# jpedro1992/gym-loadbalancing

Hardware: AMD Instinct MI355X
Metric: env-steps/sec (whole node) at 1M envs, 1/2/4/8 GPUs; % HBM roofline (higher is better)
Workload: dtype f64

## Files before the change

### gym-loadbalancing_amd/csrc/lbk8s_env.hip

```cpp

#include <hip/hip_runtime.h>

#include <cstdint>
#include <cstdio>
#include <cstdlib>
#include <algorithm>
#include <cstring>
#include <string>
#include <type_traits>

#include "lbk8s.h"
#include "lbk8s_common.h"
#include "lbk8s_host.h"
#include "lbk8s_slice.h"
#include "lbk8s_tpe.h"
#include "lbk8s_rollout.h"
#include "lbk8s_lean_launch.h"

namespace lbk {

__global__ void k_luts(double* lat_lut, double* cpu_lut) {
    int row = blockIdx.x * blockDim.x + threadIdx.x;
    if (row < LAT_ROWS) {
        double v = (double)row;
// ... 96 lines not shown
        case LB_FIELD_ENDPOINT_LATENCY: v = lat_of(p, p.lat0[i], ed); break;
        case LB_FIELD_ENDPOINT_CPU: v = cpu_of(p, em, ed); break;
        case LB_FIELD_ENDPOINT_TOPOLOGY_LATENCY: v = (double)topo_val(topo, em_zone(em), s.rz); break;
        case LB_FIELD_ENDPOINT_ZONE_CPU_CAPACITY: v = (double)zcap_val(zc, em_zone(em)); break;
        case LB_FIELD_ENDPOINT_ZONE: v = (double)em_zone(em); break;
        case LB_FIELD_ENDPOINT_NODE: v = (double)em_node(em); break;
        default: v = (double)ed_j(ed); break;
        }
        out[env * p.E + e] = v;
    }
}

__global__ void k_stats(Params p, double* out) {
    int64_t env = (int64_t)blockIdx.x * blockDim.x + threadIdx.x;
    if (env >= p.B) return;
    write_stats_row(p, out + env * LB_ST_K, sc_unpack(p.sc[env]), p.acc2[env], p.acc3[env], p.total[env],
                    p.sum_lat[env], p.sum_cpu[env], p.sum_hi[env]);
}

__global__ void k_status(Params p, uint32_t* flags) {
    int64_t env = (int64_t)blockIdx.x * blockDim.x + threadIdx.x;
    uint32_t f = 0;
    if (env < p.B) {
        Scal s = sc_unpack(p.sc[env]);
        if (s.bad) f |= LB_STATUS_BAD_ACTION;
        if (!s.reset_done) f |= LB_STATUS_NOT_RESET;
    }
    if (f) atomicOr(flags, f);
}

thread_local std::string g_err;
#ifdef LB_EXPERIMENTS
int g_rollout_variant = 0;
#else
constexpr int g_rollout_variant = 0;
#endif

int fail(const char* msg) {
    g_err = msg;
    return -1;
}

Geo geometry(const lb_config* c, int64_t B) {
    Geo g;
    const int E = c->num_endpoints;
    g.tpe = E <= TPE_E;
    if (g.tpe && B > 0 && B < WIDE_SLICE_MAX_B) g.tpe = false;
    if (E <= TPE_E && c->geometry == LB_GEOMETRY_TPE) g.tpe = true;
    if (c->geometry == LB_GEOMETRY_SLICE) g.tpe = false;
    if (g.tpe) {
        g.W = 1;
        g.EPL = 1;
        g.EP = E;
    } else {
        const bool wide = B < WIDE_SLICE_MAX_B;
        if (wide) {
            g.W = E <= 16 ? 16 : E <= 32 ? 32 : 64;
            g.EPL = E <= 64 ? 1 : E <= 128 ? 2 : 4;
        } else {
            g.W = E <= 64 ? 16 : E <= 128 ? 32 : 64;
            g.EPL = E <= 16 ? 1 : E <= 32 ? 2 : 4;
        }
        g.EP = g.W * g.EPL;
    }
    g.NZW = (c->num_nodes + 31) / 32;
    return g;
}

uint64_t align_up(uint64_t x) { return (x + 255) & ~(uint64_t)255; }

Offsets offsets(const lb_config* c, int64_t B) {
    Geo g = geometry(c, B);
    Offsets o;
    uint64_t x = 0;
    auto take = [&](uint64_t bytes) { uint64_t r = x; x = align_up(x + bytes); return r; };
    o.lat_lut = take((uint64_t)LAT_ROWS * JCAP * 8);
    o.cpu_lut = take((uint64_t)CPU_ROWS * JCAP * 8);
    const uint64_t BE = (uint64_t)B * g.EP;
    o.lat0 = take(BE * 8);
    o.emeta = take(BE * 4);
    o.edyn = take(BE * 4);
    o.t = take(B * 8);
    o.sc = take(B * 8);
    o.topo = take(B * 8);
    o.zcap = take(B * 8);
    o.nzone = take((uint64_t)B * g.NZW * 8);
    o.acc2 = take(B * 8);
    o.acc3 = take(B * 8);
    o.sum_lat = take(B * 8);
    o.sum_cpu = take(B * 8);
    o.sum_hi = take(B * 4);
    o.total = take(B * 8);
    o.last_r = take(B * 8);
    o.rew64 = take(B * 8);
    o.rec = take(g.tpe ? (uint64_t)B * RO_REC_BYTES : 0);
    o.end = x;
    return o;
}

double initial_last_reward(const lb_config* c) {
    switch (c->reward_fn) {
    case LB_REWARD_NAIVE: return 1.0;
    case LB_REWARD_LATENCY: return -(0.0 + 0.0);
    case LB_REWARD_FAIRNESS: return 1.0 - 0.0;
    default: {
        volatile double cur = ((0.0 + 0.0) - 2.0) / 998.0;
        volatile double cpu = (1.0 - 1.0) / 99.0;
        volatile double a = c->latency_weight * (1.0 - cur);
        volatile double b = c->cpu_weight * (1.0 - cpu);
        volatile double g = c->gini_weight * (1.0 - 0.0);
        volatile double ab = a + b;
        return ab + g;
    }
    }
}

int validate(const lb_config* c) {
    if (!c) return fail("lb_config is NULL");
    if (c->num_endpoints < 1 || c->num_endpoints > EMAX) return fail("num_endpoints must be in [1, 256]");
    if (c->num_zones < 4)
        return fail("IndexError: num_zones < 4 (zone ids are drawn in [0,4), loadbalancer_k8s_env.py:354)");
    if (c->num_nodes < 24)
        return fail("IndexError: num_nodes < 24 (endpoint hosts are drawn in [0,24), loadbalancer_k8s_env.py:380)");
    if (c->num_nodes > 32 * NZW_MAX) return fail("num_nodes must be <= 256");
    if (c->episode_length < 1 || c->episode_length > CMAX) return fail("episode_length must be in [1, 1023]");
    if (c->reward_fn < 0 || c->reward_fn > 3) return fail("unknown reward_fn");
    if (c->rng_mode != LB_RNG_PHILOX && c->rng_mode != LB_RNG_TRACE) return fail("unknown rng_mode");
    if (c->geometry < LB_GEOMETRY_AUTO || c->geometry > LB_GEOMETRY_SLICE) return fail("unknown geometry");
// ... 81 lines not shown
int rollout_kernel(const lb_config* c, int64_t B, int32_t steps, bool outputs_all) {
    const Geo g = geometry(c, B);
    if (!g.tpe) return LB_ROLLOUT_SLICE;
    if (g.NZW > 2) return LB_ROLLOUT_STEPS;
    const bool pre = c->auto_reset && c->episode_length >= steps;
    if (!pre) return LB_ROLLOUT_TPE;
    const uint64_t lim = 0xFFFFFFFFull;
    const int R = c->num_endpoints + (c->rejection_allowed ? 1 : 0);
    const bool img_fits = offsets(c, B).end <= lim && (uint64_t)B * LB_ST_K * 8 <= lim;
    const bool lean_fits = img_fits && (uint64_t)B * R * 32 <= lim;
    const bool lean_shape = (c->num_endpoints == 8 && R == 9 && c->num_nodes <= 32) ||
                            (c->num_endpoints == 6 && R == 7 && c->num_nodes <= 64);
    if (lean_fits && lean_shape && B % 64 == 0 && B > SMALL_TPE_MAX_B && outputs_all &&
        g_rollout_variant == 0)
        return steps <= LEAN_SPLIT_MAX_K ? LB_ROLLOUT_LEAN_SPLIT : LB_ROLLOUT_LEAN;
    if (img_fits && g_rollout_variant != 3) return LB_ROLLOUT_IMG;
    return LB_ROLLOUT_TPE;
}

template <typename F>
void with_policy(int policy, bool flag, F f) {
    auto two = [&](auto kind) {
        if (flag) f(kind, std::true_type{});
        else f(kind, std::false_type{});
    };
    switch (policy) {
    case LB_POLICY_TOPOLOGY_GREEDY: two(std::integral_constant<int, LB_POLICY_TOPOLOGY_GREEDY>{}); break;
    case LB_POLICY_ZONE_CPU_GREEDY: two(std::integral_constant<int, LB_POLICY_ZONE_CPU_GREEDY>{}); break;
    case LB_POLICY_ENDPOINT_CPU_GREEDY: two(std::integral_constant<int, LB_POLICY_ENDPOINT_CPU_GREEDY>{}); break;
    default: two(std::integral_constant<int, LB_POLICY_RANDOM>{}); break;
    }
}

}

using namespace lbk;

extern "C" {

int lb_abi_version(void) { return LBK8S_ABI_VERSION; }


#ifdef LB_EXPERIMENTS
int lbx_set_rollout_variant(int v) { g_rollout_variant = v; return 0; }
#endif
#ifdef LB_TIMELINE
int lbx_set_timeline(uint64_t* buf) {
    int r = hipMemcpyToSymbol(HIP_SYMBOL(g_timeline), &buf, sizeof(buf)) == hipSuccess ? 0 : -1;
    r |= lbx_set_timeline_lean_0(buf) | lbx_set_timeline_lean_1(buf) | lbx_set_timeline_lean_2(buf) |
         lbx_set_timeline_lean_3(buf);
    return r;
}
#endif

const char* lb_last_error(void) { return g_err.c_str(); }

int lb_validate_config(const lb_config* cfg) { return validate(cfg); }

int lb_state_bytes(const lb_config* cfg, int64_t num_envs, uint64_t* out_bytes) {
    if (int r = validate(cfg)) return r;
    if (num_envs < 1 || !out_bytes) return fail("num_envs must be >= 1 and out_bytes non-NULL");
    *out_bytes = offsets(cfg, num_envs).end;
    return 0;
}

int lb_init(void* state, const lb_config* cfg, int64_t num_envs, const lb_trace* trace, void* stream) {
    if (int r = validate(cfg)) return r;
    if (!state || num_envs < 1) return fail("state NULL or num_envs < 1");
    const bool tr = cfg->rng_mode == LB_RNG_TRACE;
    if (tr && (!trace || !trace->t0)) return fail("trace mode: lb_init needs trace->t0");
    Params p = make_params(state, cfg, num_envs);
    if (tr) p.tr = *trace;
    hipStream_t s = (hipStream_t)stream;
    hipLaunchKernelGGL(k_luts, dim3((LAT_ROWS + CPU_ROWS + 127) / 128), dim3(128), 0, s, p.lat_lut, p.cpu_lut);
    if (int r = check_launch()) return r;
    hipLaunchKernelGGL(k_init, dim3(env_blocks(num_envs)), dim3(BLOCK), 0, s, p, tr ? 1 : 0);
    return check_launch();
}

int lb_reset(void* state, const lb_config* cfg, int64_t num_envs, const uint8_t* reset_mask,
             float* obs_out, const lb_trace* trace, void* stream) {
    if (int r = validate(cfg)) return r;
    if (!state || num_envs < 1) return fail("state NULL or num_envs < 1");
    const bool tr = cfg->rng_mode == LB_RNG_TRACE;
    if (tr && (!trace || !trace->reset_lat0 || !trace->reset_topo || !trace->reset_ntype ||
               !trace->reset_nzone || !trace->reset_ncpu || !trace->reset_enode || !trace->reset_x1 ||
               !trace->reset_x2 || !trace->reset_r || !trace->reset_n))
        return fail("trace mode: lb_reset needs every reset_* trace array");
    Params p = make_params(state, cfg, num_envs);
    if (tr) p.tr = *trace;
    p.obs = obs_out;
    p.reset_mask = reset_mask;
    Geo g = geometry(cfg, num_envs);
    hipStream_t s = (hipStream_t)stream;
    if (g.tpe) {
        if (num_envs <= SMALL_TPE_MAX_B) {
            const unsigned nb = (unsigned)((num_envs + 63) / 64);
            if (tr) hipLaunchKernelGGL((k_reset_tpe<true, 64>), dim3(nb), dim3(64), 0, s, p);
            else hipLaunchKernelGGL((k_reset_tpe<false, 64>), dim3(nb), dim3(64), 0, s, p);
            return check_launch();
        }
        if (tr) hipLaunchKernelGGL(k_reset_tpe<true>, dim3(env_blocks(num_envs)), dim3(BLOCK), 0, s, p);
        else hipLaunchKernelGGL(k_reset_tpe<false>, dim3(env_blocks(num_envs)), dim3(BLOCK), 0, s, p);
        return check_launch();
    }
    LB_DISPATCH_SLICE(g.W, g.EPL, {
// ... 36 lines not shown
        } else if (tr) {
            hipLaunchKernelGGL((k_step_tpe<true, false>), dim3(env_blocks(num_envs)), dim3(BLOCK), 0, s, p);
        } else if (recompute) {
            hipLaunchKernelGGL((k_step_tpe<false, true>), dim3(env_blocks(num_envs)), dim3(BLOCK), 0, s, p);
        } else {
            hipLaunchKernelGGL((k_step_tpe<false, false>), dim3(env_blocks(num_envs)), dim3(BLOCK), 0, s, p);
        }
        return check_launch();
    }
    LB_DISPATCH_SLICE(g.W, g.EPL, {
        const unsigned nb = slice_blocks(num_envs, W);
        if (tr) hipLaunchKernelGGL((k_step_slice<W, EPL, true>), dim3(nb), dim3(BLOCK), 0, s, p);
        else hipLaunchKernelGGL((k_step_slice<W, EPL, false>), dim3(nb), dim3(BLOCK), 0, s, p);
    });
    return check_launch();
}

int lb_reward64(void* state, const lb_config* cfg, int64_t num_envs, double** out) {
    if (int r = validate(cfg)) return r;
    if (!state || num_envs < 1 || !out) return fail("state/out NULL or num_envs < 1");
    *out = make_params(state, cfg, num_envs).rew64;
    return 0;
}

int lb_rollout_kernel(const lb_config* cfg, int64_t num_envs, int32_t steps, int32_t outputs_all,
                      int32_t* kernel_out) {
    if (int r = validate(cfg)) return r;
    if (num_envs < 1 || steps < 0 || !kernel_out) return fail("num_envs < 1, steps < 0 or kernel_out NULL");
    if (cfg->rng_mode != LB_RNG_PHILOX) return fail("lb_rollout draws in Philox mode only");
    *kernel_out = rollout_kernel(cfg, num_envs, steps, outputs_all != 0);
    return 0;
}

int lb_rollout(void* state, const lb_config* cfg, int64_t num_envs, int32_t policy, int32_t steps,
               float* obs_out, float* reward_out, uint8_t* done_out, int32_t* actions_out,
               float* terminal_obs_out, double* ep_stats_out, void* stream) {
    if (int r = validate(cfg)) return r;
    if (!state || num_envs < 1) return fail("state NULL or num_envs < 1");
    if (cfg->rng_mode != LB_RNG_PHILOX) return fail("lb_rollout draws in Philox mode only");
    if (policy < 0 || policy > LB_POLICY_REWARD_GREEDY) return fail("unknown policy kind");
    if (steps < 0) return fail("steps must be >= 0");
    const bool k8s = policy > LB_POLICY_RANDOM;
    Geo g = geometry(cfg, num_envs);
    hipStream_t s = (hipStream_t)stream;
    if (g.tpe && g.NZW <= 2) {
        Params p = make_params(state, cfg, num_envs);
        p.obs = obs_out;
        p.reward = reward_out;
        p.done = done_out;
        p.term_obs = terminal_obs_out;
        p.ep_stats = ep_stats_out;
        const bool small = num_envs <= SMALL_TPE_MAX_B;
        const dim3 grid(small ? (unsigned)((num_envs + 63) / 64) : env_blocks(num_envs)), block(small ? 64 : BLOCK);
        const bool pre = cfg->auto_reset && cfg->episode_length >= steps;
        if (k8s) return launch_rollout_k8s(p, g, policy, (int)steps, pre, actions_out, s);
        const int rk = rollout_kernel(cfg, num_envs, steps, obs_out && reward_out && done_out && terminal_obs_out &&
                                                                ep_stats_out);
        if (rk == LB_ROLLOUT_LEAN || rk == LB_ROLLOUT_LEAN_SPLIT) {
            const bool naive = p.reward_fn == LB_REWARD_NAIVE, act = actions_out != nullptr;
            with_policy(policy, p.E == 8, [&](auto kind, auto e8) {
                constexpr int KIND = decltype(kind)::value, ET = decltype(e8)::value ? 8 : 6, RT = ET + 1,
                              NZW = decltype(e8)::value ? 1 : 2;
                if (naive && act) launch_lean<KIND, ET, RT, NZW, true, true>(p, num_envs, (int)steps, actions_out, s);
                else if (naive) launch_lean<KIND, ET, RT, NZW, true, false>(p, num_envs, (int)steps, actions_out, s);
                else if (act) launch_lean<KIND, ET, RT, NZW, false, true>(p, num_envs, (int)steps, actions_out, s);
                else launch_lean<KIND, ET, RT, NZW, false, false>(p, num_envs, (int)steps, actions_out, s);
            });
            return check_launch();
        }
        if (rk == LB_ROLLOUT_IMG) {
            const bool e8 = p.E == 8 && p.R == 9;
            with_policy(policy, small, [&](auto kind, auto sm) {
                constexpr int KIND = decltype(kind)::value, NB = decltype(sm)::value ? 64 : BLOCK;
                if (e8) hipLaunchKernelGGL((k_rollout_img<NB, KIND, 8, 9, 4>), grid, block, 0, s, p, (int)steps, actions_out);
                else hipLaunchKernelGGL((k_rollout_img<NB, KIND, 0, 0, 4>), grid, block, 0, s, p, (int)steps, actions_out);
            });
            return check_launch();
        }
        with_policy(policy, small, [&](auto kind, auto sm) {
            constexpr int KIND = decltype(kind)::value, NB = decltype(sm)::value ? 64 : BLOCK;
            if (pre) hipLaunchKernelGGL((k_rollout_tpe<NB, KIND, true>), grid, block, 0, s, p, (int)steps, actions_out);
            else hipLaunchKernelGGL((k_rollout_tpe<NB, KIND, false>), grid, block, 0, s, p, (int)steps, actions_out);
        });
        return check_launch();
    }
    if (g.tpe) {
        if (policy != LB_POLICY_RANDOM && !actions_out)
            return fail("lb_rollout on the thread-per-env layout needs actions_out for a greedy policy");
        const int64_t R = cfg->num_endpoints + (cfg->rejection_allowed ? 1 : 0);
        for (int k = 0; k < steps; ++k) {
            int32_t* act = actions_out ? actions_out + k * num_envs : nullptr;
            if (act)
                if (int r = lb_policy(state, cfg, num_envs, policy, act, stream)) return r;
            if (int r = lb_step(state, cfg, num_envs, act, obs_out ? obs_out + k * num_envs * R * 8 : nullptr,
                                reward_out ? reward_out + k * num_envs : nullptr,
                                done_out ? done_out + k * num_envs : nullptr, terminal_obs_out, ep_stats_out,
                                nullptr, stream))
                return r;
        }
// ... 73 lines not shown
```

### gym-loadbalancing_amd/csrc/lbk8s_host.h

```cpp
#pragma once

#include <hip/hip_runtime.h>

#include <cstdint>
#include <string>

#include "lbk8s.h"
#include "lbk8s_common.h"

namespace lbk {

extern thread_local std::string g_err;
int fail(const char* msg);
int check_launch();
int validate(const lb_config* c);

struct Geo {
    bool tpe;
    int W, EPL, EP, NZW;
};

constexpr int64_t WIDE_SLICE_MAX_B = 32768;
constexpr int64_t SMALL_TPE_MAX_B = 65536;

Geo geometry(const lb_config* c, int64_t B = 0);

struct Offsets {
    uint64_t lat_lut, cpu_lut, lat0, emeta, edyn, t, sc, topo, zcap, nzone, acc2, acc3, sum_lat,
        sum_cpu, sum_hi, total, last_r, rew64, rec, end;
};

Offsets offsets(const lb_config* c, int64_t B);
Params make_params(void* state, const lb_config* c, int64_t B);

#define LB_DISPATCH_SLICE(W_, EPL_, BODY)                                         \
    do {                                                                          \
        if (W_ == 16 && EPL_ == 1) { constexpr int W = 16, EPL = 1; BODY; }       \
        else if (W_ == 16 && EPL_ == 2) { constexpr int W = 16, EPL = 2; BODY; }  \
        else if (W_ == 16 && EPL_ == 4) { constexpr int W = 16, EPL = 4; BODY; }  \
        else if (W_ == 32 && EPL_ == 4) { constexpr int W = 32, EPL = 4; BODY; }  \
        else if (W_ == 32 && EPL_ == 1) { constexpr int W = 32, EPL = 1; BODY; }  \
        else if (W_ == 64 && EPL_ == 1) { constexpr int W = 64, EPL = 1; BODY; }  \
        else if (W_ == 64 && EPL_ == 2) { constexpr int W = 64, EPL = 2; BODY; }  \
        else if (W_ == 64 && EPL_ == 4) { constexpr int W = 64, EPL = 4; BODY; }  \
        else return fail("unsupported geometry");                                 \
    } while (0)

unsigned slice_blocks(int64_t B, int W);
unsigned env_blocks(int64_t B);
int device_cus();

int launch_policy_reward_greedy(const Params& p, const Geo& g, int32_t* actions_out, hipStream_t s);
int launch_rollout_k8s(const Params& p, const Geo& g, int policy, int steps, bool pre, int32_t* actions_out,
                       hipStream_t s);

unsigned ds_grid_spread(int64_t groups);

}
```

### gym-loadbalancing_amd/csrc/lbk8s_lean.h

```cpp
#pragma once

#include "lbk8s_rollout.h"

namespace lbk {

typedef __amdgpu_buffer_rsrc_t Rsrc;
typedef uint32_t u32x2 __attribute__((ext_vector_type(2)));
typedef uint32_t u32x4 __attribute__((ext_vector_type(4)));

__device__ __forceinline__ Rsrc rsrc_of(const void* base) {
    return __builtin_amdgcn_make_buffer_rsrc(const_cast<void*>(base), (short)0, -1, 0x00020000);
}
constexpr int BUF_NT = 2;

#define LB_GUARD_S(...) asm volatile("" : "+s"(__VA_ARGS__))
#define LB_GUARD_V(...) asm volatile("" : "+v"(__VA_ARGS__))

__device__ __forceinline__ double buf_ld_f64(Rsrc r, uint32_t off) {
    return __builtin_bit_cast(double, __builtin_amdgcn_raw_buffer_load_b64(r, off, 0, 0));
}
__device__ __forceinline__ uint4 buf_ld_u128(Rsrc r, uint32_t off) {
    const u32x4 v = __builtin_amdgcn_raw_buffer_load_b128(r, off, 0, 0);
    return make_uint4(v.x, v.y, v.z, v.w);
}
// ... 429 lines not shown
            ++cep;
        }
        if (k + 1 < K) split_draws<KIND>(p, env0 + lane, cep, cs, sst, (k + 1) & 1, lane);
        block_lds_sync();
        float4 v[CW][P];
        uint32_t rw[CW], dn[CW], ac[CW];
#pragma unroll
        for (int c = 0; c < CW; ++c) {
#pragma unroll
            for (int it = 0; it < P; ++it) v[c][it] = lean_piece<P>(simg[c], lane, it, h);
            rw[c] = sst[192 * c + lane];
            dn[c] = sst[192 * c + 64 + lane];
            ac[c] = ACT ? sst[192 * c + 128 + lane] : 0u;
        }
        block_lds_sync();
        const Rsrc out = rsrc_of(p.obs + (int64_t)k * p.B * (P / 2) * 8);
        const Rsrc rwo = rsrc_of(p.reward + (int64_t)k * p.B), dno = rsrc_of(p.done + (int64_t)k * p.B);
#pragma unroll
        for (int c = 0; c < CW; ++c) {
            const uint32_t envi = (uint32_t)(env0 + 64 * c + lane);
            const uint32_t obs_wave = (uint32_t)((env0 + 64 * c) * P * 16);
#pragma unroll
            for (int it = 0; it < P; ++it)
                buf_st_f4<BUF_NT>(v[c][it], out, (uint32_t)lane * 16u + obs_wave + 1024u * (uint32_t)it);
            __builtin_amdgcn_raw_buffer_store_b32(rw[c], rwo, envi * 4u, 0, BUF_NT);
            __builtin_amdgcn_raw_buffer_store_b8((uint8_t)dn[c], dno, envi, 0, BUF_NT);
            if (ACT) __builtin_amdgcn_raw_buffer_store_b32(ac[c], rsrc_of(act_out + (int64_t)k * p.B), envi * 4u, 0, 0);
        }
    }
}

template <int KIND, int ET, int RT, int NZW, bool NAIVE, bool ACT, int CW>
__device__ __forceinline__ void lean_body(Params p, int K, int32_t* act_out, uint32_t (*simg)[64 * IMG_W],
                                          uint32_t* sstage) {
    static_assert(CW == 0 || CW == 1, "one env wave per copy wave (two: the copy wave's registers for both blocks spilled)");
    constexpr bool SPLIT = CW > 0;
    constexpr int NB = SPLIT ? 64 * (CW + 1) : LEAN_NB, NW = SPLIT ? CW : NB / 64, P = 2 * RT, GT = 64 / P;
    constexpr int FAST = GT < REC_FETCH_MAX ? GT : REC_FETCH_MAX;
    static_assert(ET >= 1 && ET <= TPE_E && (RT == ET || RT == ET + 1), "compile-time geometry");
    (void)NW;
    const LDims<ET, RT> d(p);
    const int lane = threadIdx.x & 63, wv = threadIdx.x >> 6;
    const int64_t blk = blockIdx.x;
    if constexpr (SPLIT) {
        if (wv == CW) {
            lean_copier<P, ACT, CW, KIND>(p, K, act_out, simg, sstage, blk * 64 * CW);
            return;
        }
    }
    uint32_t* wimg = simg[wv];
    uint32_t* me = wimg + lane * IMG_W;
    const int64_t env0 = blk * (SPLIT ? 64 * CW : NB) + __builtin_amdgcn_readfirstlane(threadIdx.x & ~63);
    if (env0 >= p.B) return;
    LB_LTL_HDR(2);
    LB_LTL_HWID();
    const int64_t env = env0 + lane;
    const uint32_t envi = (uint32_t)env;
    const Rsrc blob = rsrc_of(p.lat_lut);
    const uint32_t rec_off = (uint32_t)(reinterpret_cast<const char*>(p.rec) - reinterpret_cast<const char*>(p.lat_lut));
    const uint32_t cpu0 = (uint32_t)(reinterpret_cast<const char*>(p.cpu_lut) - reinterpret_cast<const char*>(p.lat_lut));

    LEnv v;
    uint32_t em[TPE_E], ed[TPE_E];
    double l0s[TPE_E];
    {
        const uint64_t sc = p.sc[env];
        v.acc3 = p.acc3[env];
        v.s0 = (uint32_t)sc;
        v.s1 = (uint32_t)(sc >> 32);
#pragma unroll
        for (int e = 0; e < TPE_E; ++e) {
            em[e] = 0u;
            ed[e] = 0u;
            l0s[e] = 0.0;
            if (e < ET) {
                const int64_t i = (int64_t)e * p.B + env;
// ... 277 lines not shown
    }
    int64_t ew = env;
    asm volatile("" : "+v"(ew));
#pragma unroll
    for (int e = 0; e < TPE_E; ++e)
        if (e < ET) p.edyn[(int64_t)e * p.B + ew] = ed[e];
    if (new_episode) {
        const uint32_t* w = reinterpret_cast<const uint32_t*>(p.rec + ew * (RO_REC_BYTES / 16));
#pragma unroll
        for (int e = 0; e < TPE_E; ++e) {
            if (e >= ET) continue;
            const int64_t i = (int64_t)e * p.B + ew;
            p.lat0[i] = __longlong_as_double((long long)((uint64_t)w[24 + 2 * e] | ((uint64_t)w[25 + 2 * e] << 32)));
            p.emeta[i] = w[e];
        }
        p.topo[ew] = v.topo;
        p.zcap[ew] = (uint64_t)w[10] | ((uint64_t)w[11] << 32);
        p.nzone[ew] = v.nz0;
        if (NZW > 1 && p.NZW > 1) p.nzone[p.B + ew] = v.nz1;
    }
    p.t[ew] = v.t;
    p.sc[ew] = (uint64_t)v.s0 | ((uint64_t)v.s1 << 32);
    p.acc2[ew] = v.acc2;
    p.acc3[ew] = v.acc3;
    p.sum_lat[ew] = v.sum_lat;
    p.sum_cpu[ew] = v.sum_cpu;
    p.sum_hi[ew] = v.sum_hi;
    p.total[ew] = v.total;
    if (!NAIVE) p.last_r[ew] = v.last_r;
    LB_LTL_HDR(3);
}

template <int KIND, int ET, int RT, int NZW, bool NAIVE, bool ACT>
__global__ __launch_bounds__(LEAN_NB, 4) void k_rollout_lean(Params p, int K, int32_t* act_out) {
    __shared__ __attribute__((aligned(16))) uint32_t simg[LEAN_NB / 64][64 * IMG_W];
    lean_body<KIND, ET, RT, NZW, NAIVE, ACT, 0>(p, K, act_out, simg, nullptr);
}
template <int KIND, int ET, int RT, int NZW, bool NAIVE, bool ACT, int CW>
__global__ __launch_bounds__(64 * (CW + 1), 4) void k_rollout_lean_split(Params p, int K,
                                                                                       int32_t* act_out) {
    __shared__ __attribute__((aligned(16))) uint32_t simg[CW][64 * IMG_W];
    __shared__ __attribute__((aligned(16))) uint32_t sstage[CW * 3 * 64 + 2 * SD_BUF / 4];
    lean_body<KIND, ET, RT, NZW, NAIVE, ACT, CW>(p, K, act_out, simg, sstage);
}

}
```

### gym-loadbalancing_amd/csrc/lbk8s_lean_inst.hip

```cpp
#include "lbk8s_lean.h"
#include "lbk8s_lean_launch.h"

#ifndef LB_LEAN_KIND
#error "LB_LEAN_KIND (the policy of this unit) must be defined"
#endif

namespace lbk {

template <int KIND, int ET, int RT, int NZW, bool NAIVE, bool ACT>
void launch_lean(const Params& p, int64_t B, int steps, int32_t* act, hipStream_t s) {
    if (steps <= LEAN_SPLIT_MAX_K) {
        hipLaunchKernelGGL((k_rollout_lean_split<KIND, ET, RT, NZW, NAIVE, ACT, 1>), dim3((unsigned)(B / 64)), dim3(128), 0,
                           s, p, steps, act);
        return;
    }
    hipLaunchKernelGGL((k_rollout_lean<KIND, ET, RT, NZW, NAIVE, ACT>), dim3((unsigned)((B + LEAN_NB - 1) / LEAN_NB)),
                       dim3(LEAN_NB), 0, s, p, steps, act);
}

#define LB_LEAN_INST(NAIVE_, ACT_)                                                                                  \
    template void launch_lean<LB_LEAN_KIND, 8, 9, 1, NAIVE_, ACT_>(const Params&, int64_t, int, int32_t*, hipStream_t); \
    template void launch_lean<LB_LEAN_KIND, 6, 7, 2, NAIVE_, ACT_>(const Params&, int64_t, int, int32_t*, hipStream_t);
LB_LEAN_INST(true, true)
LB_LEAN_INST(true, false)
LB_LEAN_INST(false, true)
LB_LEAN_INST(false, false)
#undef LB_LEAN_INST

}

#ifdef LB_TIMELINE
#define LB_CAT2(a, b) a##b
#define LB_CAT(a, b) LB_CAT2(a, b)
extern "C" int LB_CAT(lbx_set_timeline_lean_, LB_LEAN_KIND)(uint64_t* buf) {
    return hipMemcpyToSymbol(HIP_SYMBOL(lbk::g_timeline), &buf, sizeof(buf)) == hipSuccess ? 0 : -1;
}
#endif
```

### gym-loadbalancing_amd/csrc/lbk8s_lean_launch.h

```cpp
#pragma once

#include <hip/hip_runtime.h>

#include "lbk8s_common.h"

namespace lbk {

constexpr int LEAN_SPLIT_MAX_K = 32;

template <int KIND, int ET, int RT, int NZW, bool NAIVE, bool ACT>
void launch_lean(const Params& p, int64_t B, int steps, int32_t* act, hipStream_t s);

#define LB_LEAN_EXTERN(KIND_, NAIVE_, ACT_)                                                                    \
    extern template void launch_lean<KIND_, 8, 9, 1, NAIVE_, ACT_>(const Params&, int64_t, int, int32_t*, hipStream_t); \
    extern template void launch_lean<KIND_, 6, 7, 2, NAIVE_, ACT_>(const Params&, int64_t, int, int32_t*, hipStream_t);
#define LB_LEAN_EXTERN_KIND(KIND_)                                                                             \
    LB_LEAN_EXTERN(KIND_, true, true) LB_LEAN_EXTERN(KIND_, true, false) LB_LEAN_EXTERN(KIND_, false, true)     \
    LB_LEAN_EXTERN(KIND_, false, false)
LB_LEAN_EXTERN_KIND(0)
LB_LEAN_EXTERN_KIND(1)
LB_LEAN_EXTERN_KIND(2)
LB_LEAN_EXTERN_KIND(3)
#undef LB_LEAN_EXTERN_KIND
#undef LB_LEAN_EXTERN

}

#ifdef LB_TIMELINE
extern "C" int lbx_set_timeline_lean_0(uint64_t* buf);
extern "C" int lbx_set_timeline_lean_1(uint64_t* buf);
extern "C" int lbx_set_timeline_lean_2(uint64_t* buf);
extern "C" int lbx_set_timeline_lean_3(uint64_t* buf);
#endif
```

### gym-loadbalancing_amd/lbk8s/_native.py

```python
import ctypes as C
import os

LIB_PATH = os.path.join(os.path.dirname(os.path.abspath(__file__)), "liblbk8s.so")
_PRODUCT_LIB = LIB_PATH
CSRC = os.path.join(os.path.dirname(os.path.dirname(os.path.abspath(__file__))), "csrc")
SOURCES = ("lbk8s_env_steps.hip", "lbk8s_env.hip", "lbk8s_ds.hip", "lbk8s_ds_train.hip", "lbk8s_steps.hip",
           "lbk8s_learn.hip", "lbk8s_host.h", "lbk8s_common.h", "lbk8s_slice.h", "lbk8s_tpe.h", "lbk8s_rollout.h", "lbk8s_lean.h",
           "lbk8s_deepsets.h", "lbk8s_ds_train.h", "lbk8s_steps.h", "lbk8s_dqn.h", "lbk8s_ppo.h", "lbk8s_eval.h",
           "../../include/lbk8s.h", "../../include/lbk8s_abi_steps64.h", "../../include/lbk8s_abi_dqn64.h",
           "../../include/lbk8s_abi_steps256.h", "../../include/lbk8s_abi_dqn256.h", "lbk8s_lean_launch.h", "lbk8s_lean_inst.hip", "lbk8s_policies.hip", "lbk8s_steps64.h", "lbk8s_dqn64.h",
           "lbk8s_steps64.hip", "lbk8s_steps256.h", "lbk8s_dqn256.h", "lbk8s_steps256.hip", "lbk8s_steps_host.h",
           "lbk8s_build.cpp")
ABI_VERSION = 17

LB_REWARD = {"naive": 0, "latency": 1, "fairness": 2, "multi": 3}
LB_RNG_PHILOX, LB_RNG_TRACE = 0, 1
LB_POLICY = {"topo": 0, "zone_cpu": 1, "endpoint_cpu": 2, "random": 3,
             "round_robin": 4, "least_loaded": 5, "least_latency": 6, "reward_greedy": 7}
POLICIES_WITHOUT_LEAN_KERNELS = ("round_robin", "least_loaded", "least_latency", "reward_greedy")
LB_DS_FWD, LB_DS_FWD_TRAIN, LB_DS_FWD_ARGMAX, LB_DS_FWD_PAIR, LB_DS_FWD_SAMPLE = 0, 1, 2, 3, 5
LB_ROLLOUT = {0: "k_rollout_lean", 1: "k_rollout_img", 2: "k_rollout_tpe", 3: "policy+step launches",
              4: "k_rollout_slice", 5: "k_rollout_lean_split"}
LB_FIELD = {"endpoint_latency": 0, "endpoint_cpu_usage_percentage": 1,
            "endpoint_topology_latency": 2, "endpoint_zone_cpu_capacity": 3, "endpoint_zone": 4,
            "endpoint_node": 5, "avg_load_served": 6, "current_time": 7, "current_step": 8,
            "request_zone": 9, "request_threshold": 10}
PER_ENV_FIELDS = {"current_time", "current_step", "request_zone", "request_threshold"}
LB_ST_K = 16
LB_EPLOG_W = 24
LB_EPLOG_RET32, LB_EPLOG_REWARD, LB_EPLOG_ACTION, LB_EPLOG_ENV, LB_EPLOG_TAG = 16, 17, 18, 19, 20
LB_STATUS_BAD_ACTION, LB_STATUS_NOT_RESET = 1, 2
LB_PPO_STEPS_MAX = 4096
LB_EVAL_STEPS_MAX = 4096
LB_GEOMETRY = {"auto": 0, "tpe": 1, "slice": 2}


class LBConfigC(C.Structure):
    _fields_ = [("num_endpoints", C.c_int32), ("num_zones", C.c_int32), ("num_nodes", C.c_int32),
                ("episode_length", C.c_int32), ("reward_fn", C.c_int32),
                ("rejection_allowed", C.c_int32), ("auto_reset", C.c_int32), ("rng_mode", C.c_int32),
                ("arrival_rate", C.c_double), ("call_duration", C.c_double),
                ("latency_weight", C.c_double), ("cpu_weight", C.c_double),
                ("gini_weight", C.c_double), ("seed", C.c_uint64), ("env_id_offset", C.c_int64),
# ... 80 lines not shown
        "lb_eval_steps_supported": [cfgp, i64, i32],
        "lb_eval_steps": [vp, vp, vp, cfgp, i64, i32, vp, i32] + [vp] * 11 + log_tail,
        "lb_ds_train_forward": [vp, vp, i64, i32] + [vp] * 6,
        "lb_ds_forward_pair": [vp] * 8 + [i64, i32, vp],
        "lb_ds_forward_kernel": [i32, i64, i32, i32p, i32p, i32p],
        "lb_ppo_head": [vp] * 8 + [i64, i32, f32, f32, f32, i32, vp, vp, vp, vp],
        "lb_ds_pack_backward": [wp, vp, vp],
        "lb_ds_pack_pair": [wp, vp, vp, vp],
        "lb_ds_train_backward": [vp, vp, i64, i32] + [vp] * 8,
        "lb_ds_set_grads": [vp, vp, vp, i64, i32, vp, vp],
        "lb_ds_train_backward_sets": [vp, vp, i64, i32] + [vp] * 9,
        "lb_ds_over_sets": [C.POINTER(LBSetJobC), i32, i64, vp, i64, vp],
    }
    protos = {name: (C.c_int, args) for name, args in ints.items()}
    for name in ("lb_last_error", "lb_source_hash", "lb_build_flags", "lb_build_compiler"):
        protos[name] = (C.c_char_p, [])
    return protos


PROTOTYPES = _prototypes()
EXPORTED_SYMBOLS = tuple(PROTOTYPES)
STEPS64_PROTOTYPES = {name.replace("_steps", "_steps64"): PROTOTYPES[name]
                      for name in ("lb_ppo_steps_supported", "lb_ppo_steps", "lb_eval_steps_supported", "lb_eval_steps")}
STEPS64_SYMBOLS = tuple(STEPS64_PROTOTYPES)
DQN64_PROTOTYPES = {name.replace("_steps", "_steps64"): PROTOTYPES[name]
                    for name in ("lb_dqn_steps_supported", "lb_dqn_steps")}
DQN64_SYMBOLS = tuple(DQN64_PROTOTYPES)
STEPS256_PROTOTYPES = {name.replace("_steps", "_steps256"): PROTOTYPES[name]
                       for name in ("lb_eval_steps_supported", "lb_eval_steps")}
STEPS256_SYMBOLS = tuple(STEPS256_PROTOTYPES)
DQN256_PROTOTYPES = {name.replace("_steps", "_steps256"): PROTOTYPES[name]
                     for name in ("lb_dqn_steps_supported", "lb_dqn_steps")}
DQN256_SYMBOLS = tuple(DQN256_PROTOTYPES)

_lib = None


class NativeLibraryMissing(RuntimeError):
    pass


class StaleNativeLibrary(RuntimeError):
    pass


class NonDefaultBuild(StaleNativeLibrary):
    """A product library compiled with other flags than csrc/Makefile's defaults (a -D knob of
    a diagnostic build, another optimisation level): refused like a stale one."""


class _Tolerant:

    class _Missing:
        def __init__(self, name):
            self.name = name

        def __call__(self, *a):
            raise AttributeError(f"diagnostic library lacks {self.name}")

    def __init__(self, L):
        self.__dict__["_L"] = L

    def __getattr__(self, name):
        try:
            return getattr(self._L, name)
        except AttributeError:
# ... 26 lines not shown
def expected_build_flags():
    path = os.path.join(CSRC, "Makefile")
    if not os.path.exists(path):
        return None
    with open(path) as fh:
        text = fh.read()
    flags = _makefile_var(text, "HIPFLAGS").replace("$(ARCH)", _makefile_var(text, "ARCH"))
    return " ".join(flags.split())


def build_hash(L):
    import hashlib
    parts = [L.lb_source_hash(), L.lb_build_flags(), L.lb_build_compiler()]
    return hashlib.sha256(b"\n".join(parts)).hexdigest()[:16]


def lib():
    global _lib
    if _lib is not None:
        return _lib
    import torch
    if not os.path.exists(LIB_PATH):
        raise NativeLibraryMissing(
            f"{LIB_PATH} not found: build it with `make -C gym-loadbalancing_amd/csrc` "
            "(or __graft_entry__.build()); there is no CPU fallback")
    L = C.CDLL(LIB_PATH)
    product = os.path.abspath(LIB_PATH) == _PRODUCT_LIB
    if not product:
        L = _Tolerant(L)
    for name, (restype, argtypes) in PROTOTYPES.items():
        f = getattr(L, name)
        f.restype, f.argtypes = restype, argtypes
    for name, (restype, argtypes) in {**STEPS64_PROTOTYPES, **DQN64_PROTOTYPES, **STEPS256_PROTOTYPES,
                                       **DQN256_PROTOTYPES}.items():
        if hasattr(L, name):
            f = getattr(L, name)
            f.restype, f.argtypes = restype, argtypes
    v = L.lb_abi_version()
    if v != ABI_VERSION and product:
        raise RuntimeError(f"liblbk8s.so ABI {v} != expected {ABI_VERSION}; rebuild it")
    if product:
        built, now = L.lb_source_hash().decode(), source_hash()
        if now is not None and built != now:
            raise StaleNativeLibrary(f"{LIB_PATH} was built from sources {built}, the tree's are {now}: "
                                     "rebuild it (make -C gym-loadbalancing_amd/csrc, or __graft_entry__.build())")
        flags, want = " ".join(L.lb_build_flags().decode().split()), expected_build_flags()
        if want is not None and flags != want:
            raise NonDefaultBuild(f"{LIB_PATH} was built with flags '{flags}', csrc/Makefile's defaults are "
                                  f"'{want}': a diagnostic build is not the product (rebuild with make -B)")
    _lib = L
    return L


def check(rc):
    if rc == 0:
        return
    msg = lib().lb_last_error().decode()
    if msg.startswith("IndexError"):
        raise IndexError(msg)
    raise RuntimeError(f"liblbk8s: {msg} (rc={rc})")
```

### gym-loadbalancing_amd/lbk8s/vec_env.py

```python
import ctypes as C
import csv
import json
import os
import time

import numpy as np

from . import _native
from .config import LBConfig
from .info import ST_ACC, ST_EPISODE, ST_LENGTH, ST_RETURN, csv_rows, step_info

_TRACE_SPEC = {
    "t0": ("f8", None), "step_x1": ("f8", None), "step_x2": ("f8", None), "step_r": ("i4", None),
    "step_n": ("i4", None), "reset_lat0": ("f8", "E"), "reset_topo": ("i4", "ZZ"),
    "reset_ntype": ("i4", "N"), "reset_nzone": ("i4", "N"), "reset_ncpu": ("i4", "N"),
    "reset_enode": ("i4", "E"), "reset_x1": ("f8", None), "reset_x2": ("f8", None),
    "reset_r": ("i4", None), "reset_n": ("i4", None),
}


class LazyInfos:

    def __init__(self, env, rewards, actions, dones, monitor_t):
        self._env, self._r, self._a, self._d = env, rewards, actions, dones
# ... 495 lines not shown
        if not self._reset_called:
            raise TypeError("step() called before reset()")
        _native.check(self._L.lb_step(
            self._ptr(self.state), C.byref(self._c), self.num_envs, self._ptr(actions),
            self._ptr(obs_out if obs_out is not None else self.obs),
            self._ptr(reward_out if reward_out is not None else self.rewards),
            self._ptr(done_out if done_out is not None else self.dones),
            self._ptr(terminal_obs_out if terminal_obs_out is not None else self.terminal_obs),
            self._ptr(ep_stats_out if ep_stats_out is not None else self.ep_stats),
            C.byref(self._trace) if self.trace_mode else None, self._stream()))

    def rollout(self, kind, steps, obs_out=None, reward_out=None, done_out=None, actions_out=None,
                terminal_obs_out=None, ep_stats_out=None):
        if not self._reset_called:
            raise TypeError("step() called before reset()")
        if self.trace_mode:
            raise RuntimeError("rollout() draws from Philox; trace mode steps one call at a time")
        _native.check(self._L.lb_rollout(
            self._ptr(self.state), C.byref(self._c), self.num_envs, _native.LB_POLICY[kind], int(steps),
            self._ptr(obs_out), self._ptr(reward_out), self._ptr(done_out), self._ptr(actions_out),
            self._ptr(terminal_obs_out if terminal_obs_out is not None else self.terminal_obs),
            self._ptr(ep_stats_out if ep_stats_out is not None else self.ep_stats), self._stream()))

    def rollout_kernel(self, steps, outputs_all=True, kind=None):
        k = C.c_int32(-1)
        _native.check(self._L.lb_rollout_kernel(C.byref(self._c), self.num_envs, int(steps), int(bool(outputs_all)),
                                                C.byref(k)))
        name = _native.LB_ROLLOUT[k.value]
        lean = ("k_rollout_lean", "k_rollout_lean_split", "k_rollout_img")
        if kind in _native.POLICIES_WITHOUT_LEAN_KERNELS and name in lean:
            return "k_rollout_tpe"
        return name

    def policy(self, kind, out=None):
        out = out if out is not None else self.torch.empty(self.num_envs, dtype=self.torch.int32,
                                                           device=self.device)
        _native.check(self._L.lb_policy(self._ptr(self.state), C.byref(self._c), self.num_envs,
                                        _native.LB_POLICY[kind], self._ptr(out), self._stream()))
        return out

    def dqn_act(self, frag, obs, masks, ex, out):
        R = obs.shape[1]
        _native.check(self._L.lb_dqn_act(frag.data_ptr(), obs.data_ptr(), self.num_envs, R, self._ptr(masks),
                                         self._ptr(self.state), C.byref(self._c), C.byref(ex), self._ptr(out),
                                         self._stream()))
        return out

    def dqn_step(self, frag, obs, masks, ex, actions, next_obs, reward, done, rb, pos_in, pos_out, ep_sum, ep_cnt):
        self._dqn_guard()
        _native.check(self._L.lb_dqn_step(
            *self._dqn_args(frag, obs, masks, ex, actions, next_obs, reward, done, rb, pos_in, pos_out, ep_sum, ep_cnt),
            self._stream()))
        return actions

    def _dqn_args(self, frag, obs, masks, ex, actions, next_obs, reward, done, rb, pos_in, pos_out, ep_sum, ep_cnt):
        return (frag.data_ptr(), obs.data_ptr(), self.num_envs, obs.shape[1], self._ptr(masks), self._ptr(self.state),
                C.byref(self._c), C.byref(ex), self._ptr(actions), self._ptr(next_obs), self._ptr(reward),
                self._ptr(done), self._ptr(self.terminal_obs), self._ptr(self.ep_stats), rb.size, pos_in, pos_out,
                rb.obs.data_ptr(), rb.next_obs.data_ptr(), rb.actions.data_ptr(), rb.rewards.data_ptr(),
                rb.dones.data_ptr(), self._ptr(ep_sum), self._ptr(ep_cnt))

    def _dqn_guard(self):
        if not self._reset_called and not self.torch.cuda.is_current_stream_capturing():
            raise TypeError("step() called before reset()")
        if self.trace_mode:
            raise RuntimeError("the DQN step draws its exploration and actions from Philox; trace mode steps "
# ... 87 lines not shown
```

### include/lbk8s.h

```cpp
#ifndef LBK8S_H
#define LBK8S_H

#include <stddef.h>
#include <stdint.h>

#ifdef __cplusplus
extern "C" {
#endif

#define LBK8S_ABI_VERSION 17

enum { LB_REWARD_NAIVE = 0, LB_REWARD_LATENCY = 1, LB_REWARD_FAIRNESS = 2, LB_REWARD_MULTI = 3 };
enum { LB_RNG_PHILOX = 0, LB_RNG_TRACE = 1 };
enum {
    LB_POLICY_TOPOLOGY_GREEDY = 0,
    LB_POLICY_ZONE_CPU_GREEDY = 1,
    LB_POLICY_ENDPOINT_CPU_GREEDY = 2,
    LB_POLICY_RANDOM = 3,
    LB_POLICY_ROUND_ROBIN = 4,
    LB_POLICY_LEAST_LOADED = 5,
    LB_POLICY_LEAST_LATENCY = 6,
    LB_POLICY_REWARD_GREEDY = 7
};
enum {
// ... 264 lines not shown

int lb_ds_train_backward(const float* bwd_frag, const float* obs, int64_t num_envs, int32_t num_elements,
                         const float* save_actor, const float* save_critic, const float* dlogits,
                         const float* dmean, float* wgrad_out, float* workspace, float* setvec,
                         void* stream);

#define LB_DS_SETGRAD_ACTOR 4736
#define LB_DS_SETGRAD_CRITIC 12800
int lb_ds_set_grads(const float* setvec, const float* dlogits, const float* dmean, int64_t num_sets,
                    int32_t num_elements, float* out, void* stream);

int lb_ds_train_backward_sets(const float* bwd_frag, const float* obs, int64_t num_envs, int32_t num_elements,
                              const float* save_actor, const float* save_critic, const float* dlogits,
                              const float* dmean, float* wgrad_out, float* workspace, float* setvec,
                              float* set_grads_out, void* stream);

#define LB_DS_OVER_SETS_SPAN 256
typedef struct lb_set_job {
    const float* a;
    int64_t lda;
    const float* b;
    int64_t ldb;
    int32_t M, N;
    float scale;
    float* out;
} lb_set_job;
int lb_ds_over_sets(const lb_set_job* jobs, int32_t num_jobs, int64_t num_sets, float* workspace,
                    int64_t workspace_floats, void* stream);

#include "lbk8s_abi_steps64.h"
#include "lbk8s_abi_dqn64.h"
#include "lbk8s_abi_steps256.h"
#include "lbk8s_abi_dqn256.h"

#ifdef __cplusplus
}
#endif

#endif
```

Before: 19.92 billion.

## Add ticket-based dynamic block scheduling to lean rollout kernels

Result: no change. 20.16 billion, median of 6 (+1.2%).

```diff
diff --git a/gym-loadbalancing_amd/csrc/lbk8s_env.hip b/gym-loadbalancing_amd/csrc/lbk8s_env.hip
--- a/gym-loadbalancing_amd/csrc/lbk8s_env.hip
+++ b/gym-loadbalancing_amd/csrc/lbk8s_env.hip
@@ -152,8 +152,12 @@
 thread_local std::string g_err;
 #ifdef LB_EXPERIMENTS
 int g_rollout_variant = 0;
+int64_t g_lean_gt_max = -1;
+int g_lean_f4 = LEAN_TICKET_F4;
 #else
 constexpr int g_rollout_variant = 0;
+constexpr int64_t g_lean_gt_max = -1;
+constexpr int g_lean_f4 = LEAN_TICKET_F4;
 #endif
 
 int fail(const char* msg) {
@@ -214,6 +218,7 @@
     o.last_r = take(B * 8);
     o.rew64 = take(B * 8);
     o.rec = take(g.tpe ? (uint64_t)B * RO_REC_BYTES : 0);
+    o.ticket = take(4);
     o.end = x;
     return o;
 }
@@ -361,6 +366,18 @@
     }
 }
 
+template <typename F>
+void with_lean(const Params& p, int policy, bool act, F f) {
+    const bool naive = p.reward_fn == LB_REWARD_NAIVE;
+    with_policy(policy, p.E == 8, [&](auto kind, auto e8) {
+        using ET = std::integral_constant<int, decltype(e8)::value ? 8 : 6>;
+        if (naive && act) f(kind, ET{}, std::true_type{}, std::true_type{});
+        else if (naive) f(kind, ET{}, std::true_type{}, std::false_type{});
+        else if (act) f(kind, ET{}, std::false_type{}, std::true_type{});
+        else f(kind, ET{}, std::false_type{}, std::false_type{});
+    });
+}
+
 }
 
 using namespace lbk;
@@ -372,6 +389,11 @@
 
 #ifdef LB_EXPERIMENTS
 int lbx_set_rollout_variant(int v) { g_rollout_variant = v; return 0; }
+int lbx_set_lean_deal(int64_t gt_max, int f4) {
+    g_lean_gt_max = gt_max;
+    g_lean_f4 = f4 < 4 ? 4 : f4;
+    return 0;
+}
 #endif
 #ifdef LB_TIMELINE
 int lbx_set_timeline(uint64_t* buf) {
@@ -401,6 +423,8 @@
     Params p = make_params(state, cfg, num_envs);
     if (tr) p.tr = *trace;
     hipStream_t s = (hipStream_t)stream;
+    if (hipMemsetAsync((char*)state + offsets(cfg, num_envs).ticket, 0, sizeof(uint32_t), s) != hipSuccess)
+        return fail("hipMemsetAsync failed");
     hipLaunchKernelGGL(k_luts, dim3((LAT_ROWS + CPU_ROWS + 127) / 128), dim3(128), 0, s, p.lat_lut, p.cpu_lut);
     if (int r = check_launch()) return r;
     hipLaunchKernelGGL(k_init, dim3(env_blocks(num_envs)), dim3(BLOCK), 0, s, p, tr ? 1 : 0);
@@ -503,6 +527,31 @@
     return 0;
 }
 
+int lb_lean_ticket_split(const void* state, const lb_config* cfg, int64_t num_envs, int32_t policy, int32_t steps,
+                         int32_t with_actions, int64_t* static_out, int64_t* ticketed_out, int64_t* grid_out) {
+    if (!state) return fail("lb_lean_ticket_split: state NULL");
+    if (int r = validate(cfg)) return r;
+    if (num_envs < 1 || steps < 0 || !static_out || !ticketed_out || !grid_out)
+        return fail("lb_lean_ticket_split: num_envs < 1, steps < 0 or an output NULL");
+    if (cfg->rng_mode != LB_RNG_PHILOX) return fail("lb_lean_ticket_split: lb_rollout draws in Philox mode only");
+    if (policy < 0 || policy > LB_POLICY_RANDOM)
+        return fail("lb_lean_ticket_split: no lean kernel for this policy kind");
+    const int rk = rollout_kernel(cfg, num_envs, steps, true);
+    if (rk != LB_ROLLOUT_LEAN && rk != LB_ROLLOUT_LEAN_SPLIT)
+        return fail("lb_lean_ticket_split: lb_rollout takes no lean kernel at this shape (ask lb_rollout_kernel)");
+    const Params p = make_params(const_cast<void*>(state), cfg, num_envs);
+    with_lean(p, policy, with_actions != 0, [&](auto kind, auto et, auto naive, auto ac) {
+        constexpr int KIND = decltype(kind)::value, ET = decltype(et)::value, RT = ET + 1, NZW = ET == 8 ? 1 : 2;
+        const LeanDeal d = lean_deal(num_envs / 64,
+                                     lean_resident<KIND, ET, RT, NZW, decltype(naive)::value, decltype(ac)::value>((int)steps),
+                                     g_lean_gt_max, g_lean_f4);
+        *static_out = d.n_static;
+        *ticketed_out = d.n_ticketed;
+        *grid_out = d.grid;
+    });
+    return 0;
+}
+
 int lb_rollout(void* state, const lb_config* cfg, int64_t num_envs, int32_t policy, int32_t steps,
                float* obs_out, float* reward_out, uint8_t* done_out, int32_t* actions_out,
                float* terminal_obs_out, double* ep_stats_out, void* stream) {
@@ -528,14 +577,14 @@
         const int rk = rollout_kernel(cfg, num_envs, steps, obs_out && reward_out && done_out && terminal_obs_out &&
                                                                 ep_stats_out);
         if (rk == LB_ROLLOUT_LEAN || rk == LB_ROLLOUT_LEAN_SPLIT) {
-            const bool naive = p.reward_fn == LB_REWARD_NAIVE, act = actions_out != nullptr;
-            with_policy(policy, p.E == 8, [&](auto kind, auto e8) {
-                constexpr int KIND = decltype(kind)::value, ET = decltype(e8)::value ? 8 : 6, RT = ET + 1,
-                              NZW = decltype(e8)::value ? 1 : 2;
-                if (naive && act) launch_lean<KIND, ET, RT, NZW, true, true>(p, num_envs, (int)steps, actions_out, s);
-                else if (naive) launch_lean<KIND, ET, RT, NZW, true, false>(p, num_envs, (int)steps, actions_out, s);
-                else if (act) launch_lean<KIND, ET, RT, NZW, false, true>(p, num_envs, (int)steps, actions_out, s);
-                else launch_lean<KIND, ET, RT, NZW, false, false>(p, num_envs, (int)steps, actions_out, s);
+            const bool act = actions_out != nullptr;
+            uint32_t* ticket = (uint32_t*)((char*)state + offsets(cfg, num_envs).ticket);
+            with_lean(p, policy, act, [&](auto kind, auto et, auto naive, auto ac) {
+                constexpr int KIND = decltype(kind)::value, ET = decltype(et)::value, RT = ET + 1, NZW = ET == 8 ? 1 : 2;
+                constexpr bool NAIVE = decltype(naive)::value, ACT = decltype(ac)::value;
+                const LeanDeal d = lean_deal(num_envs / 64, lean_resident<KIND, ET, RT, NZW, NAIVE, ACT>((int)steps),
+                                             g_lean_gt_max, g_lean_f4);
+                launch_lean<KIND, ET, RT, NZW, NAIVE, ACT>(p, num_envs, (int)steps, actions_out, ticket, d, s);
             });
             return check_launch();
         }
diff --git a/gym-loadbalancing_amd/csrc/lbk8s_host.h b/gym-loadbalancing_amd/csrc/lbk8s_host.h
--- a/gym-loadbalancing_amd/csrc/lbk8s_host.h
+++ b/gym-loadbalancing_amd/csrc/lbk8s_host.h
@@ -27,7 +27,7 @@
 
 struct Offsets {
     uint64_t lat_lut, cpu_lut, lat0, emeta, edyn, t, sc, topo, zcap, nzone, acc2, acc3, sum_lat,
-        sum_cpu, sum_hi, total, last_r, rew64, rec, end;
+        sum_cpu, sum_hi, total, last_r, rew64, rec, ticket, end;
 };
 
 Offsets offsets(const lb_config* c, int64_t B);
diff --git a/gym-loadbalancing_amd/csrc/lbk8s_lean.h b/gym-loadbalancing_amd/csrc/lbk8s_lean.h
--- a/gym-loadbalancing_amd/csrc/lbk8s_lean.h
+++ b/gym-loadbalancing_amd/csrc/lbk8s_lean.h
@@ -485,7 +485,7 @@
 
 template <int KIND, int ET, int RT, int NZW, bool NAIVE, bool ACT, int CW>
 __device__ __forceinline__ void lean_body(Params p, int K, int32_t* act_out, uint32_t (*simg)[64 * IMG_W],
-                                          uint32_t* sstage) {
+                                          uint32_t* sstage, uint32_t* ticket, int n_static, int n_ticketed) {
     static_assert(CW == 0 || CW == 1, "one env wave per copy wave (two: the copy wave's registers for both blocks spilled)");
     constexpr bool SPLIT = CW > 0;
     constexpr int NB = SPLIT ? 64 * (CW + 1) : LEAN_NB, NW = SPLIT ? CW : NB / 64, P = 2 * RT, GT = 64 / P;
@@ -494,7 +494,20 @@
     (void)NW;
     const LDims<ET, RT> d(p);
     const int lane = threadIdx.x & 63, wv = threadIdx.x >> 6;
-    const int64_t blk = blockIdx.x;
+    int64_t blk = blockIdx.x;
+    if ((int)blockIdx.x >= n_static) {
+        uint32_t t = 0;
+        if constexpr (SPLIT) {
+            if (threadIdx.x == 0) sstage[0] = atomicInc(ticket, gridDim.x - (uint32_t)n_static - 1u);
+            block_lds_sync();
+            t = sstage[0];
+        } else {
+            if (lane == 0) t = atomicInc(ticket, gridDim.x - (uint32_t)n_static - 1u);
+        }
+        t = (uint32_t)__builtin_amdgcn_readfirstlane((int)t);
+        if (t >= (uint32_t)n_ticketed) return;
+        blk = (int64_t)n_static + t;
+    }
     if constexpr (SPLIT) {
         if (wv == CW) {
             lean_copier<P, ACT, CW, KIND>(p, K, act_out, simg, sstage, blk * 64 * CW);
@@ -838,16 +851,19 @@
 }
 
 template <int KIND, int ET, int RT, int NZW, bool NAIVE, bool ACT>
-__global__ __launch_bounds__(LEAN_NB, 4) void k_rollout_lean(Params p, int K, int32_t* act_out) {
+__global__ __launch_bounds__(LEAN_NB, 4) void k_rollout_lean(Params p, int K, int32_t* act_out, uint32_t* ticket,
+                                                             int n_static, int n_ticketed) {
     __shared__ __attribute__((aligned(16))) uint32_t simg[LEAN_NB / 64][64 * IMG_W];
-    lean_body<KIND, ET, RT, NZW, NAIVE, ACT, 0>(p, K, act_out, simg, nullptr);
+    lean_body<KIND, ET, RT, NZW, NAIVE, ACT, 0>(p, K, act_out, simg, nullptr, ticket, n_static, n_ticketed);
 }
 template <int KIND, int ET, int RT, int NZW, bool NAIVE, bool ACT, int CW>
 __global__ __launch_bounds__(64 * (CW + 1), 4) void k_rollout_lean_split(Params p, int K,
-                                                                                       int32_t* act_out) {
+                                                                                       int32_t* act_out,
+                                                                                       uint32_t* ticket, int n_static,
+                                                                                       int n_ticketed) {
     __shared__ __attribute__((aligned(16))) uint32_t simg[CW][64 * IMG_W];
     __shared__ __attribute__((aligned(16))) uint32_t sstage[CW * 3 * 64 + 2 * SD_BUF / 4];
-    lean_body<KIND, ET, RT, NZW, NAIVE, ACT, CW>(p, K, act_out, simg, sstage);
-}
-
-}
+    lean_body<KIND, ET, RT, NZW, NAIVE, ACT, CW>(p, K, act_out, simg, sstage, ticket, n_static, n_ticketed);
+}
+
+}
diff --git a/gym-loadbalancing_amd/csrc/lbk8s_lean_inst.hip b/gym-loadbalancing_amd/csrc/lbk8s_lean_inst.hip
--- a/gym-loadbalancing_amd/csrc/lbk8s_lean_inst.hip
+++ b/gym-loadbalancing_amd/csrc/lbk8s_lean_inst.hip
@@ -8,19 +8,45 @@
 namespace lbk {
 
 template <int KIND, int ET, int RT, int NZW, bool NAIVE, bool ACT>
-void launch_lean(const Params& p, int64_t B, int steps, int32_t* act, hipStream_t s) {
+int64_t lean_resident(int steps) {
+    auto ask = [](auto kernel, int threads) -> int64_t {
+        int dev = 0, cus = 0, per_cu = 0;
+        if (hipGetDevice(&dev) != hipSuccess ||
+            hipDeviceGetAttribute(&cus, hipDeviceAttributeMultiprocessorCount, dev) != hipSuccess ||
+            hipOccupancyMaxActiveBlocksPerMultiprocessor(&per_cu, kernel, threads, 0) != hipSuccess || cus < 1 ||
+            per_cu < 1) {
+            (void)hipGetLastError();
+            return 0;
+        }
+        return (int64_t)cus * per_cu;
+    };
     if (steps <= LEAN_SPLIT_MAX_K) {
-        hipLaunchKernelGGL((k_rollout_lean_split<KIND, ET, RT, NZW, NAIVE, ACT, 1>), dim3((unsigned)(B / 64)), dim3(128), 0,
-                           s, p, steps, act);
+        static const int64_t r = ask(k_rollout_lean_split<KIND, ET, RT, NZW, NAIVE, ACT, 1>, 128);
+        return r;
+    }
+    static const int64_t r = ask(k_rollout_lean<KIND, ET, RT, NZW, NAIVE, ACT>, LEAN_NB);
+    return r;
+}
+
+template <int KIND, int ET, int RT, int NZW, bool NAIVE, bool ACT>
+void launch_lean(const Params& p, int64_t B, int steps, int32_t* act, uint32_t* ticket, const LeanDeal& d, hipStream_t s) {
+    (void)B;
+    if (steps <= LEAN_SPLIT_MAX_K) {
+        hipLaunchKernelGGL((k_rollout_lean_split<KIND, ET, RT, NZW, NAIVE, ACT, 1>), dim3((unsigned)d.grid), dim3(128), 0, s,
+                           p, steps, act, ticket, (int)d.n_static, (int)d.n_ticketed);
         return;
     }
-    hipLaunchKernelGGL((k_rollout_lean<KIND, ET, RT, NZW, NAIVE, ACT>), dim3((unsigned)((B + LEAN_NB - 1) / LEAN_NB)),
-                       dim3(LEAN_NB), 0, s, p, steps, act);
+    hipLaunchKernelGGL((k_rollout_lean<KIND, ET, RT, NZW, NAIVE, ACT>), dim3((unsigned)d.grid), dim3(LEAN_NB), 0, s, p,
+                       steps, act, ticket, (int)d.n_static, (int)d.n_ticketed);
 }
 
 #define LB_LEAN_INST(NAIVE_, ACT_)                                                                                  \
-    template void launch_lean<LB_LEAN_KIND, 8, 9, 1, NAIVE_, ACT_>(const Params&, int64_t, int, int32_t*, hipStream_t); \
-    template void launch_lean<LB_LEAN_KIND, 6, 7, 2, NAIVE_, ACT_>(const Params&, int64_t, int, int32_t*, hipStream_t);
+    template void launch_lean<LB_LEAN_KIND, 8, 9, 1, NAIVE_, ACT_>(const Params&, int64_t, int, int32_t*, uint32_t*, \
+                                                                   const LeanDeal&, hipStream_t);                   \
+    template void launch_lean<LB_LEAN_KIND, 6, 7, 2, NAIVE_, ACT_>(const Params&, int64_t, int, int32_t*, uint32_t*, \
+                                                                   const LeanDeal&, hipStream_t);                   \
+    template int64_t lean_resident<LB_LEAN_KIND, 8, 9, 1, NAIVE_, ACT_>(int);                                       \
+    template int64_t lean_resident<LB_LEAN_KIND, 6, 7, 2, NAIVE_, ACT_>(int);
 LB_LEAN_INST(true, true)
 LB_LEAN_INST(true, false)
 LB_LEAN_INST(false, true)
diff --git a/gym-loadbalancing_amd/csrc/lbk8s_lean_launch.h b/gym-loadbalancing_amd/csrc/lbk8s_lean_launch.h
--- a/gym-loadbalancing_amd/csrc/lbk8s_lean_launch.h
+++ b/gym-loadbalancing_amd/csrc/lbk8s_lean_launch.h
@@ -8,12 +8,31 @@
 
 constexpr int LEAN_SPLIT_MAX_K = 32;
 
+struct LeanDeal {
+    int64_t n_static, n_ticketed, grid;
+};
+constexpr int LEAN_TICKET_F4 = 5;
+inline LeanDeal lean_deal(int64_t G, int64_t R, int64_t gt_max = -1, int f4 = LEAN_TICKET_F4) {
+    if (R < 1 || G <= R) return {G, 0, G};
+    int64_t gt = G - R;
+    if (gt_max >= 0 && gt > gt_max) gt = gt_max;
+    if (gt == 0) return {G, 0, G};
+    return {G - gt, gt, G - gt + (f4 * gt + 3) / 4};
+}
+
 template <int KIND, int ET, int RT, int NZW, bool NAIVE, bool ACT>
-void launch_lean(const Params& p, int64_t B, int steps, int32_t* act, hipStream_t s);
+int64_t lean_resident(int steps);
+
+template <int KIND, int ET, int RT, int NZW, bool NAIVE, bool ACT>
+void launch_lean(const Params& p, int64_t B, int steps, int32_t* act, uint32_t* ticket, const LeanDeal& d, hipStream_t s);
 
 #define LB_LEAN_EXTERN(KIND_, NAIVE_, ACT_)                                                                    \
-    extern template void launch_lean<KIND_, 8, 9, 1, NAIVE_, ACT_>(const Params&, int64_t, int, int32_t*, hipStream_t); \
-    extern template void launch_lean<KIND_, 6, 7, 2, NAIVE_, ACT_>(const Params&, int64_t, int, int32_t*, hipStream_t);
+    extern template void launch_lean<KIND_, 8, 9, 1, NAIVE_, ACT_>(const Params&, int64_t, int, int32_t*, uint32_t*, \
+                                                                   const LeanDeal&, hipStream_t);              \
+    extern template void launch_lean<KIND_, 6, 7, 2, NAIVE_, ACT_>(const Params&, int64_t, int, int32_t*, uint32_t*, \
+                                                                   const LeanDeal&, hipStream_t);              \
+    extern template int64_t lean_resident<KIND_, 8, 9, 1, NAIVE_, ACT_>(int);                                  \
+    extern template int64_t lean_resident<KIND_, 6, 7, 2, NAIVE_, ACT_>(int);
 #define LB_LEAN_EXTERN_KIND(KIND_)                                                                             \
     LB_LEAN_EXTERN(KIND_, true, true) LB_LEAN_EXTERN(KIND_, true, false) LB_LEAN_EXTERN(KIND_, false, true)     \
     LB_LEAN_EXTERN(KIND_, false, false)
diff --git a/gym-loadbalancing_amd/lbk8s/_native.py b/gym-loadbalancing_amd/lbk8s/_native.py
--- a/gym-loadbalancing_amd/lbk8s/_native.py
+++ b/gym-loadbalancing_amd/lbk8s/_native.py
@@ -8,7 +8,8 @@
            "lbk8s_learn.hip", "lbk8s_host.h", "lbk8s_common.h", "lbk8s_slice.h", "lbk8s_tpe.h", "lbk8s_rollout.h", "lbk8s_lean.h",
            "lbk8s_deepsets.h", "lbk8s_ds_train.h", "lbk8s_steps.h", "lbk8s_dqn.h", "lbk8s_ppo.h", "lbk8s_eval.h",
            "../../include/lbk8s.h", "../../include/lbk8s_abi_steps64.h", "../../include/lbk8s_abi_dqn64.h",
-           "../../include/lbk8s_abi_steps256.h", "../../include/lbk8s_abi_dqn256.h", "lbk8s_lean_launch.h", "lbk8s_lean_inst.hip", "lbk8s_policies.hip", "lbk8s_steps64.h", "lbk8s_dqn64.h",
+           "../../include/lbk8s_abi_steps256.h", "../../include/lbk8s_abi_dqn256.h",
+           "../../include/lbk8s_abi_lean_ticket.h", "lbk8s_lean_launch.h", "lbk8s_lean_inst.hip", "lbk8s_policies.hip", "lbk8s_steps64.h", "lbk8s_dqn64.h",
            "lbk8s_steps64.hip", "lbk8s_steps256.h", "lbk8s_dqn256.h", "lbk8s_steps256.hip", "lbk8s_steps_host.h",
            "lbk8s_build.cpp")
 ABI_VERSION = 17
@@ -155,6 +156,9 @@
 DQN256_PROTOTYPES = {name.replace("_steps", "_steps256"): PROTOTYPES[name]
                      for name in ("lb_dqn_steps_supported", "lb_dqn_steps")}
 DQN256_SYMBOLS = tuple(DQN256_PROTOTYPES)
+LEAN_TICKET_PROTOTYPES = {"lb_lean_ticket_split": (C.c_int, [C.c_void_p, C.POINTER(LBConfigC), C.c_int64, C.c_int32,
+                                                             C.c_int32, C.c_int32] + [C.POINTER(C.c_int64)] * 3)}
+LEAN_TICKET_SYMBOLS = tuple(LEAN_TICKET_PROTOTYPES)
 
 _lib = None
 
@@ -247,7 +251,7 @@
         f = getattr(L, name)
         f.restype, f.argtypes = restype, argtypes
     for name, (restype, argtypes) in {**STEPS64_PROTOTYPES, **DQN64_PROTOTYPES, **STEPS256_PROTOTYPES,
-                                       **DQN256_PROTOTYPES}.items():
+                                       **DQN256_PROTOTYPES, **LEAN_TICKET_PROTOTYPES}.items():
         if hasattr(L, name):
             f = getattr(L, name)
             f.restype, f.argtypes = restype, argtypes
diff --git a/gym-loadbalancing_amd/lbk8s/vec_env.py b/gym-loadbalancing_amd/lbk8s/vec_env.py
--- a/gym-loadbalancing_amd/lbk8s/vec_env.py
+++ b/gym-loadbalancing_amd/lbk8s/vec_env.py
@@ -551,6 +551,13 @@
             return "k_rollout_tpe"
         return name
 
+    def lean_ticket_split(self, steps, kind="random", actions=False):
+        out = [C.c_int64(-1) for _ in range(3)]
+        _native.check(self._L.lb_lean_ticket_split(self._ptr(self.state), C.byref(self._c), self.num_envs,
+                                                   _native.LB_POLICY[kind], int(steps), int(bool(actions)),
+                                                   *[C.byref(o) for o in out]))
+        return tuple(o.value for o in out)
+
     def policy(self, kind, out=None):
         out = out if out is not None else self.torch.empty(self.num_envs, dtype=self.torch.int32,
                                                            device=self.device)
diff --git a/include/lbk8s.h b/include/lbk8s.h
--- a/include/lbk8s.h
+++ b/include/lbk8s.h
@@ -320,6 +320,7 @@
 #include "lbk8s_abi_dqn64.h"
 #include "lbk8s_abi_steps256.h"
 #include "lbk8s_abi_dqn256.h"
+#include "lbk8s_abi_lean_ticket.h"
 
 #ifdef __cplusplus
 }
diff --git a/include/lbk8s_abi_lean_ticket.h b/include/lbk8s_abi_lean_ticket.h
--- /dev/null
+++ b/include/lbk8s_abi_lean_ticket.h
@@ -0,0 +1,7 @@
+#ifndef LBK8S_ABI_LEAN_TICKET_H
+#define LBK8S_ABI_LEAN_TICKET_H
+
+int lb_lean_ticket_split(const void* state, const lb_config* cfg, int64_t num_envs, int32_t policy, int32_t steps,
+                         int32_t with_actions, int64_t* static_out, int64_t* ticketed_out, int64_t* grid_out);
+
+#endif
```
